# danieleschmidt/spin-torque-rl-gym

Hardware: AMD Instinct MI355X
Metric: env_steps_per_sec (higher is better)
Workload: dtype f64

## Files before the change

### spin-torque-rl-gym_amd/csrc/stg_kernels.hpp

```cpp
#pragma once
#include "../../include/spintorque_hip.h"
#include "stg_launch_plan.hpp"
#include "stg_physics.hpp"

#include <hip/hip_runtime.h>

#include <type_traits>

using namespace stg;

struct alignas(16) EnvRec {
    double m[3];
    double tgt[3];
    double etot;
    uint32_t stepw;
    uint32_t rng;
};
static_assert(sizeof(EnvRec) == 64, "state record size");
constexpr uint32_t STG_DONE_BIT = 0x80000000u;

struct StateView {
    EnvRec* rec;
};

// ... 557 lines not shown
            if (more && takers != 0ull) {
                const int n_take = (int)__builtin_popcountll(takers), first = (int)__builtin_ctzll(takers);
                const int rank = (int)__builtin_popcountll(takers & ((1ull << lane) - 1ull));
                const int64_t avail = loc_end - loc_q;
                const int need_new = n_take > avail ? (int)(n_take - avail) : 0;
                int64_t new_q = 0;
                const int new_stripe = stripe;
                if (need_new > 0 && queue_open) {
                    const int reserve = (takers == ~0ull && full_streak >= 1) ? 4 * 64 : need_new;
                    unsigned long long base = 0;
                    if (lane == first) base = atomicAdd(a.refill_cursor + stripe * REFILL_CURSOR_STRIDE, (unsigned long long)reserve);
                    base = (unsigned long long)__shfl((long long)base, first);
                    new_q = (int64_t)base;
                    const int64_t stripe_end = ((n_rest - stripe + REFILL_STRIPES - 1) / REFILL_STRIPES) * 64;
                    int64_t new_end = new_q + reserve;
                    if (new_end >= stripe_end) {
                        new_end = stripe_end;
                        const int64_t end_l = ((n_rest - lane + REFILL_STRIPES - 1) / REFILL_STRIPES) * 64;
                        const unsigned long long cur_l = __hip_atomic_load(a.refill_cursor + lane * REFILL_CURSOR_STRIDE, __ATOMIC_RELAXED, __HIP_MEMORY_SCOPE_AGENT);
                        unsigned long long open_s = __ballot((int64_t)cur_l < end_l);
                        open_s &= ~(1ull << stripe);
                        if (open_s == 0ull) queue_open = false;
                        else {
                            const unsigned long long after = stripe == 63 ? 0ull : (open_s >> (stripe + 1)) << (stripe + 1);
                            stripe = (int)__builtin_ctzll(after != 0ull ? after : open_s);
                        }
                    }
                    const bool from_old = rank < avail;
                    const int64_t q = from_old ? loc_q + rank : new_q + (rank - avail);
                    const int st = from_old ? loc_stripe : new_stripe;
                    const int64_t r = (q >> 6) * REFILL_STRIPES + st;
                    take((nw + r) * 64 + (q & 63), !has_env && r < n_rest && (from_old || q < new_end));
                    loc_q = new_q + need_new < new_end ? new_q + need_new : new_end;
                    loc_end = new_end;
                    loc_stripe = new_stripe;
                } else {
                    const int64_t q = loc_q + rank;
                    const int64_t r = (q >> 6) * REFILL_STRIPES + loc_stripe;
                    take((nw + r) * 64 + (q & 63), !has_env && q < loc_end && r < n_rest);
                    loc_q = loc_q + n_take < loc_end ? loc_q + n_take : loc_end;
                }
                more = queue_open || loc_q < loc_end;
                full_streak = takers == ~0ull ? full_streak + 1 : 0;
            }
        }
        if (__ballot(has_env) == 0ull && !more) break;
    }
}

template <int SOLVER, bool THERMAL, int MULTI, bool AXIS_Z, bool DEVPHYS, typename AT, bool PC, int WGW, bool IDS>
#ifndef STG_STEP_ATTR
#define STG_STEP_ATTR
#endif
__global__ void __launch_bounds__(PC ? 2 * WGW * 64 : WGW * 64, (SOLVER != STG_SOLVER_RK45 && !THERMAL && !DEVPHYS && AXIS_Z && MULTI != 2 && !(MULTI && WGW == 1)) ? 4 : 1) STG_STEP_ATTR
stg_step_kernel(const StepArgs a) {
#pragma clang fp contract(off)
    static_assert(!PC || THERMAL, "wave specialisation only exists for the thermal kernels");
    extern __shared__ double s_tab[];
    constexpr bool FIELD = SOLVER == STG_SOLVER_RK45;
    using NT = typename std::conditional<FIELD, double, float>::type;
    constexpr bool BARRIER = SOLVER != STG_SOLVER_RK4;
    constexpr int DEPTH = BARRIER ? 2 : 4;
    constexpr int RING = DEPTH * (FIELD ? SHARED_CHUNK_RK45 : SHARED_CHUNK_FIXED) * 64;
    static_assert(!PC || WGW == 1, "the wave-specialised form is one integrating + one producing wavefront");
    __shared__ NT s_norm[PC ? RING : 1];
    __shared__ int s_hs[2], s_go[2 * WGW];
    __shared__ unsigned long long s_cnt[(PC ? 2 : 1) * WGW * 3];
    __shared__ uint32_t s_rng[PC ? WGW * 64 : 1];
    const int lane = (int)(threadIdx.x & 63u);
    const int wave = __builtin_amdgcn_readfirstlane((int)(threadIdx.x >> 6));
    bool paired = PC;
    int64_t hyb_slot = 0;
    if (PC && a.hybrid) hyb_slot = stg_hybrid_block(blockIdx.x, wave, (uint32_t)(a.hybrid - 1), (a.N + TILE_ENVS - 1) / TILE_ENVS, paired);
    const bool producer = PC && paired && wave >= WGW;
    const int cw = producer ? (2 * WGW - 1 - wave) : (wave < WGW ? wave : wave - WGW);
    record_placement(a.placement, wave, lane, producer);
    const int64_t lane_slot = ((PC && a.hybrid) ? hyb_slot
                                                : stg_slot_block<WGW>(blockIdx.x, (uint32_t)((a.N + WGW * 64 - 1) / (WGW * 64)), a.perm != nullptr, cw, PC,
                                                                      (uint32_t)a.snake_rounds) * 64) + lane;
    const bool in_list = lane_slot < a.N;
    const int64_t o = in_list ? (a.perm ? (int64_t)a.perm[lane_slot] : lane_slot) : 0;
    const uint32_t id = (IDS && in_list) ? a.ids[o] : 0u;
    const bool bad = IDS && in_list && (int64_t)id >= a.n_state;
    if (bad && !producer) write_bad_id(a, o);
    const bool live = in_list && !bad;
    const int64_t i = IDS ? (live ? (int64_t)id : 0) : o;
    constexpr int ENV_LAYOUT = SOLVER == STG_SOLVER_RK45 ? ENV_LAYOUT_LLGS : (DEVPHYS ? ENV_LAYOUT_DEV : ENV_LAYOUT_CORE);
    double own_row[MULTI == 2 ? C_COUNT : 1];
    const double* row;
    if constexpr (MULTI == 2) {
        stg_device_params p;
        load_env_params<ENV_LAYOUT>(a.ep, i, p);
        derive_row(p, a.ep.gamma, a.ep.temperature, own_row);
        row = own_row;
    } else {
        row = class_row<MULTI != 0>(a.ctab, a.cls, a.ncls, i, live, s_tab, a.ep, ENV_LAYOUT);
    }
    if (!PC && !live) return;
    if (PC && !paired && !live) return;
    const int64_t N = a.N;
    const uint64_t env_id = (uint64_t)(a.env_id0 + i);

    if (producer) {
        constexpr int n_first = SOLVER == STG_SOLVER_RK45 ? SHARED_FIRST_RK45 : SHARED_CHUNK_FIXED;
        static_assert(3 * SHARED_SUBS3 == SHARED_CHUNK_FIXED, "chunk size of the 3-normal sub-steps");
        constexpr int n_chunk = SOLVER == STG_SOLVER_RK45 ? SHARED_CHUNK_RK45 : n_first;
        const double ghs = FIELD ? load_llgs(row).ghs : 0.0;
        for (int k = 0; k < a.K; ++k) {
            __syncthreads();
            const int p = (k & 1) * WGW;
            if (!any_flag<WGW>(lds_flag(s_go + p))) continue;
            const RngKey rk{a.c.seed, env_id, s_rng[cw * 64 + lane]};
            produce_normals<NT, FIELD, DEPTH, BARRIER>(s_norm, s_hs, lane, rk, n_first, n_chunk, ghs);
        }
        record_retired(a.placement, wave, lane, 0ull);
        return;
    }

    V3 m, tgt;
    double etot;
    int32_t step;
    uint32_t rng;
    bool done;
    load_state(a.s, i, m, tgt, etot, step, rng, done);
    const AT* act = (const AT*)a.actions;
    const Recorder norec{};
    unsigned long long c_steps = 0, c_sub = 0, c_noop = 0;

    for (int k = 0; k < a.K; ++k) {
        double J, T;
        if (k == 0 && a.perm) {
            typedef typename std::conditional<std::is_same<AT, double>::value, double2, float2>::type AT2;
            const AT2 aa = ((const AT2*)a.act_sorted)[live ? lane_slot : 0];
            parse_action<AT>(aa.x, aa.y, a.c.max_current, a.c.max_duration, J, T);
        } else {
            parse_action<AT>(act[((int64_t)k * 2 + 0) * N + o], act[((int64_t)k * 2 + 1) * N + o], a.c.max_current,
                             a.c.max_duration, J, T);
        }
        const bool last = (k == a.K - 1);
        const int64_t ko = a.out_every ? k : 0;
        const bool wr = (a.out_every || last) && live;
        const bool lane_solves = live && !(a.c.skip_done && done);
        const RngKey rk{a.c.seed, env_id, rng};
        SolveOut so{m, 0, 0, 0, false};
        if (PC && paired) {
            SharedNormalsT<NT, FIELD, DEPTH, BARRIER> shared{s_norm, s_hs, lane, 0, 0, 1};
            const int p = (k & 1) * WGW;
            s_rng[cw * 64 + lane] = rng;
            const bool mine = __ballot(lane_solves) != 0ull;
            s_go[p + cw] = mine ? 1 : 0;
            __syncthreads();
            if ((WGW == 1) ? mine : any_flag<WGW>(lds_flag(s_go + p))) {
                if (!BARRIER) s_hs[1] = 0;
                __syncthreads();
                so = run_solver<SOLVER, THERMAL, false, AXIS_Z, DEVPHYS>(m, J, T, row, a.c, rk, norec, shared, lane_solves);
            }
        }
        if (!(PC && paired) && lane_solves) {
            InlineNormals inl;
            so = run_solver<SOLVER, THERMAL, false, AXIS_Z, DEVPHYS>(m, J, T, row, a.c, rk, norec, inl, true);
        }
        env_step_tail(a, o, ko, wr, live, lane_solves, row, env_id, m, tgt, etot, step, rng, done, J, T, so, c_steps, c_sub, c_noop);
    }
    if (live) store_state(a.s, i, m, tgt, etot, step, rng, done);
    record_retired(a.placement, wave, lane, c_sub);
    const int ci = PC ? wave : cw;
    wave_add3(a.counters + (size_t)((blockIdx.x * (PC ? 2 : 1) * WGW + ci) % COUNTER_STRIPES) * COUNTER_STRIDE, s_cnt + ci * 3, c_steps, c_sub, c_noop);
}

template <bool THERMAL, bool MULTI, bool AXIS_Z, typename AT, int WGW, bool IDS>
__global__ void __launch_bounds__(WGW * 64) stg_step_refill_kernel(const StepArgs a) {
    extern __shared__ double s_tab[];
    __shared__ unsigned long long s_cnt[WGW * 3];
    const int lane = (int)(threadIdx.x & 63u);
    const int wave = __builtin_amdgcn_readfirstlane((int)(threadIdx.x >> 6));
    if (MULTI) {
        for (int j = threadIdx.x; j < a.ncls * C_COUNT; j += blockDim.x) s_tab[j] = a.ctab[j];
        __syncthreads();
    }
    const int64_t tiles = (a.N + TILE_ENVS - 1) / TILE_ENVS, nblk = tiles * TILE_WAVES, nw = a.refill_nw;
    const int64_t w = (int64_t)blockIdx.x * WGW + wave;
    record_placement(a.placement, wave, lane, false);
    if (w >= nw) return;
    unsigned long long c_steps = 0, c_sub = 0, c_noop = 0;
    refill_wave<THERMAL, MULTI, AXIS_Z, AT, IDS>(a, w, nw, 0, nblk, lane, s_tab, c_steps, c_sub, c_noop);
    refill_retire(a, w, nw, lane);
    record_retired(a.placement, wave, lane, c_sub);
    wave_add3(a.counters + (size_t)((blockIdx.x * WGW + wave) % COUNTER_STRIPES) * COUNTER_STRIDE, s_cnt + wave * 3, c_steps, c_sub, c_noop);
}

constexpr int64_t STG_WG4_MIN_ENVS = 65536;

template <class F>
static inline void with_flag(bool v, F&& f) {
    if (v) f(std::true_type{}); else f(std::false_type{});
}
template <class F>
static inline void with_multi(int multi, F&& f) {
    if (multi == 2) f(std::integral_constant<int, 2>{});
    else if (multi) f(std::integral_constant<int, 1>{});
    else f(std::integral_constant<int, 0>{});
}

template <int MULTI>
static size_t step_dyn_lds(const StepArgs& a) {
    return MULTI == 1 ? (size_t)a.ncls * C_COUNT * sizeof(double) : 0;
}

static inline unsigned step_grid(const StepArgs& a, int wgw) {
    const unsigned nwg = (unsigned)((a.N + wgw * 64 - 1) / (wgw * 64));
    if (!a.perm) return nwg;
    const unsigned tile_wgs = (unsigned)(TILE_WAVES / wgw);
    return ((nwg + tile_wgs - 1) / tile_wgs) * tile_wgs;
}

static int resident_workgroups_per_cu(const void* kernel, int block, size_t lds) {
    struct Key { const void* f; size_t lds; int v; };
    static thread_local Key cache[8] = {};
    static thread_local int used = 0;
    for (int j = 0; j < used; ++j) if (cache[j].f == kernel && cache[j].lds == lds) return cache[j].v;
    int nb = 0;
    if (hipOccupancyMaxActiveBlocksPerMultiprocessor(&nb, kernel, block, lds) != hipSuccess || nb < 1) nb = 2;
    if (used < 8) cache[used++] = Key{kernel, lds, nb};
    return nb;
}

static int32_t snake_rounds_of(const StepArgs& a, const void* kernel, int wgw, size_t lds) {
    if (!a.perm) return 0;
    const unsigned n_q = step_grid(a, wgw) / 8u;
    const int nb = resident_workgroups_per_cu(kernel, wgw * 64, lds);
    return (n_q > 32u && nb >= 2 && n_q <= 32u * (unsigned)nb + 16u) ? nb : 0;
}

template <int SOLVER, bool THERMAL, int MULTI, bool AXIS_Z, bool DEVPHYS, typename AT, bool PC, int WGW, bool IDS>
static void launch_step(const StepArgs& a, hipStream_t st) {
    if constexpr ((PC && (!THERMAL || DEVPHYS || WGW != 1)) || (DEVPHYS && SOLVER == STG_SOLVER_RK45)) return;
    else {
        const size_t lds = step_dyn_lds<MULTI>(a);
        StepArgs b = a;
        dim3 grid(step_grid(a, WGW));
        if constexpr (PC) {
            if (a.hybrid) grid = dim3(1024u);
            b.snake_rounds = (a.perm && step_grid(a, 1) / 8u <= 64u) ? 2 : 0;
        } else {
            b.snake_rounds = snake_rounds_of(a, (const void*)&stg_step_kernel<SOLVER, THERMAL, MULTI, AXIS_Z, DEVPHYS, AT, PC, WGW, IDS>, WGW, lds);
        }
        hipLaunchKernelGGL((stg_step_kernel<SOLVER, THERMAL, MULTI, AXIS_Z, DEVPHYS, AT, PC, WGW, IDS>), grid, dim3((PC ? 2 : 1) * WGW * 64), lds, st, b);
    }
}

template <int SOLVER, bool IDS>
static void dispatch_step(const StepArgs& a, bool thermal, int multi, bool axis_z, bool devphys, int act_f64, bool pc, hipStream_t st) {
    devphys = devphys && SOLVER != STG_SOLVER_RK45;
    pc = pc && thermal && !devphys;
    const bool wg4 = !pc && a.N >= STG_WG4_MIN_ENVS;
    with_flag(thermal, [&](auto THERMAL) { with_multi(multi, [&](auto MULTI) { with_flag(axis_z, [&](auto AXIS_Z) {
    with_flag(devphys, [&](auto DEVPHYS) { with_flag(act_f64 != 0, [&](auto F64) { with_flag(pc, [&](auto PC) { with_flag(wg4, [&](auto WG4) {
        using AT = std::conditional_t<F64.value, double, float>;
        launch_step<SOLVER, THERMAL.value, MULTI.value, AXIS_Z.value, DEVPHYS.value, AT, PC.value, WG4.value ? 4 : 1, IDS>(a, st);
    }); }); }); }); }); }); });
}

template <bool IDS>
static void dispatch_refill(const StepArgs& a, bool thermal, bool multi, bool axis_z, int act_f64, hipStream_t st) {
    constexpr int WGW = 4;
    const dim3 grid((unsigned)(((int64_t)a.refill_nw + WGW - 1) / WGW));
    with_flag(thermal, [&](auto THERMAL) { with_flag(multi, [&](auto MULTI) { with_flag(axis_z, [&](auto AXIS_Z) { with_flag(act_f64 != 0, [&](auto F64) {
        using AT = std::conditional_t<F64.value, double, float>;
        hipLaunchKernelGGL((stg_step_refill_kernel<THERMAL.value, MULTI.value, AXIS_Z.value, AT, WGW, IDS>), grid, dim3(WGW * 64),
                           step_dyn_lds<MULTI.value ? 1 : 0>(a), st, a);
    }); }); }); });
}

void stg_dispatch_step_rk4(const StepArgs& a, bool thermal, int multi, bool axis_z, bool devphys, int act_f64, bool pc, hipStream_t st);
void stg_dispatch_step_euler(const StepArgs& a, bool thermal, int multi, bool axis_z, bool devphys, int act_f64, bool pc, hipStream_t st);
void stg_dispatch_step_rk45(const StepArgs& a, bool thermal, int multi, bool axis_z, int act_f64, bool pc, hipStream_t st);
void stg_dispatch_step_rk45_refill(const StepArgs& a, bool thermal, bool multi, bool axis_z, int act_f64, hipStream_t st);
```

### spin-torque-rl-gym_amd/csrc/stg_physics.hpp

```cpp
#pragma once

#include <hip/hip_runtime.h>
#include <stdint.h>
#include <type_traits>

#include "stg_minstep.hpp"

namespace stg {

enum ClassConst : int {
    C_EX = 0, C_EY, C_EZ,
    C_HK,
    C_MS,
    C_ALPHA,
    C_GEFF,
    C_POL,
    C_MSV,
    C_HS_SIMPLE,
    C_RX, C_RY, C_RZ,
    C_DX, C_DY, C_DZ,
    C_HEX,
    C_BETA, C_BETAP,
    C_GAMMA,
    C_HS_LLGS,
// ... 71 lines not shown
#pragma clang fp contract(off)
    const double r = a - b;
    return r;
}

__device__ __forceinline__ double rsqrt_fast(double s) {
    const double y = __builtin_amdgcn_rsq(s);
    const double e = __builtin_fma(-(s * y), y, 1.0);
    return __builtin_fma(y * e, __builtin_fma(0.375, e, 0.5), y);
}

__device__ __forceinline__ void batch_ready(double at, double a0, double a1, double a2, double b0, double b1, double b2) {
    asm volatile("" : : "v"(at), "v"(a0), "v"(a1), "v"(a2), "v"(b0), "v"(b1), "v"(b2));
}

__device__ __forceinline__ double vgpr_const(double c) {
    asm volatile("" : "+v"(c));
    return c;
}

__device__ __forceinline__ double fmax_abs(double a, double b) {
    double r;
    asm("v_max_f64 %0, |%1|, |%2|" : "=v"(r) : "v"(a), "v"(b));
    return r;
}

__device__ __forceinline__ void commit_step(unsigned long long mask, double& d0, double s0, double& d1, double s1, double& d2, double s2,
                                            double& d3, double s3, double& d4, double s4, double& d5, double s5, double& d6, double s6) {
    unsigned long long saved;
    asm("s_and_saveexec_b64 %[sv], %[m]\n\t"
        "v_mov_b64 %[d0], %[s0]\n\t"
        "v_mov_b64 %[d1], %[s1]\n\t"
        "v_mov_b64 %[d2], %[s2]\n\t"
        "v_mov_b64 %[d3], %[s3]\n\t"
        "v_mov_b64 %[d4], %[s4]\n\t"
        "v_mov_b64 %[d5], %[s5]\n\t"
        "v_mov_b64 %[d6], %[s6]\n\t"
        "s_mov_b64 exec, %[sv]"
        : [d0] "+v"(d0), [d1] "+v"(d1), [d2] "+v"(d2), [d3] "+v"(d3), [d4] "+v"(d4), [d5] "+v"(d5), [d6] "+v"(d6), [sv] "=&s"(saved)
        : [s0] "v"(s0), [s1] "v"(s1), [s2] "v"(s2), [s3] "v"(s3), [s4] "v"(s4), [s5] "v"(s5), [s6] "v"(s6), [m] "s"(mask)
        : "scc");
}

__device__ __forceinline__ double rcp_fast(double x) {
    const double y = __builtin_amdgcn_rcp(x);
    return __builtin_fma(y, __builtin_fma(-x, y, 1.0), y);
}

__device__ __forceinline__ double inv_tenth_root(double e2, double tenth = 0.1) {
    const double y = (double)__builtin_amdgcn_exp2f(-0.1f * __builtin_amdgcn_logf((float)e2));
    const double y2 = y * y, y4 = y2 * y2, y8 = y4 * y4;
    const double e = __builtin_fma(-e2, y8 * y2, 1.0);
    return __builtin_fma(y * e, __builtin_fma(0.055, e, tenth), y);
}

__device__ __forceinline__ double fifth_root(double x) {
    int e;
    const double mant = frexp(x, &e);
    const double t = -0.2 * ((double)e + (double)__builtin_amdgcn_logf((float)mant));
    const double ti = rint(t);
    double r = ldexp((double)__builtin_amdgcn_exp2f((float)(t - ti)), (int)ti);
    const double r2 = r * r, r4 = r2 * r2;
    const double err = __builtin_fma(-x, r4 * r, 1.0);
    r = __builtin_fma(r * err, __builtin_fma(0.12, err, 0.2), r);
    const double q2 = r * r;
    return x * (q2 * q2);
}

__device__ __forceinline__ V3 cross(const V3& a, const V3& b) {
#pragma clang fp contract(off)
    return V3{__builtin_fma(a.y, b.z, -(a.z * b.y)), __builtin_fma(a.z, b.x, -(a.x * b.z)), __builtin_fma(a.x, b.y, -(a.y * b.x))};
}
__device__ __forceinline__ double dot(const V3& a, const V3& b) {
#pragma clang fp contract(off)
    return __builtin_fma(a.z, b.z, __builtin_fma(a.y, b.y, a.x * b.x));
}
__device__ __forceinline__ V3 scale3(double c, const V3& z) {
#pragma clang fp contract(off)
    return V3{c * z.x, c * z.y, c * z.z};
}
__device__ __forceinline__ bool finite3(const V3& a) { return isfinite(a.x) && isfinite(a.y) && isfinite(a.z); }

__device__ __forceinline__ void philox4x32_10(uint32_t c0, uint32_t c1, uint32_t c2, uint32_t c3, uint32_t k0,
                                              uint32_t k1, uint32_t (&out)[4]) {
#pragma unroll
    for (int r = 0; r < 10; ++r) {
        const uint32_t hi0 = __umulhi(0xD2511F53u, c0), lo0 = 0xD2511F53u * c0;
        const uint32_t hi1 = __umulhi(0xCD9E8D57u, c2), lo1 = 0xCD9E8D57u * c2;
        const uint32_t n0 = hi1 ^ c1 ^ k0, n2 = hi0 ^ c3 ^ k1;
        c0 = n0; c1 = lo1; c2 = n2; c3 = lo0;
        k0 += 0x9E3779B9u; k1 += 0xBB67AE85u;
    }
    out[0] = c0; out[1] = c1; out[2] = c2; out[3] = c3;
}

struct NormalStream {
    uint32_t s0, s1, s2, s3;
    float carry;
    __device__ __forceinline__ void init(uint64_t seed, uint64_t env_id, uint32_t env_step, uint32_t tag) {
        uint32_t r[4];
        philox4x32_10((uint32_t)env_id, (uint32_t)(env_id >> 32), env_step, tag, (uint32_t)seed, (uint32_t)(seed >> 32), r);
        s0 = r[0]; s1 = r[1]; s2 = r[2]; s3 = r[3] | 1u;
        carry = 0.0f;
    }
    __device__ __forceinline__ uint32_t next() {
        const uint32_t result = s0 + s3;
        const uint32_t t = s1 << 9;
        s2 ^= s0; s3 ^= s1; s1 ^= s2; s0 ^= s3; s2 ^= t;
        s3 = (s3 << 11) | (s3 >> 21);
        return result;
    }
    __device__ __forceinline__ float uniform() {
        return __uint_as_float(__builtin_amdgcn_alignbit(0x7fu, next(), 9u)) - 0.99999994f;
    }
    typedef float f32x2 __attribute__((ext_vector_type(2)));
    __device__ __forceinline__ void pair(float& a, float& b) {
        float t, c, s_;
        pair_head(t, c, s_);
        finish_pair(t, c, s_, a, b);
    }
    __device__ __forceinline__ void pair_head(float& t, float& c, float& s_) {
        f32x2 u{__uint_as_float(__builtin_amdgcn_alignbit(0x7fu, next(), 9u)), __uint_as_float(__builtin_amdgcn_alignbit(0x7fu, next(), 9u))};
        u = u - f32x2{0.99999994f, 0.99999994f};
        t = -1.3862943611198906f * __builtin_amdgcn_logf(u.x);
        c = __builtin_amdgcn_cosf(u.y);
        s_ = __builtin_amdgcn_sinf(u.y);
    }
    static __device__ __forceinline__ void finish_pair(float t, float c, float s_, float& a, float& b) {
        const float r = __builtin_amdgcn_sqrtf(t);
        const f32x2 cs = f32x2{c, s_} * f32x2{r, r};
        a = cs.x;
        b = cs.y;
    }
    __device__ __forceinline__ V3 draw3_even() {
        float a, b, c, d;
        pair(a, b);
        pair(c, d);
        carry = d;
        return V3{(double)a, (double)b, (double)c};
    }
    __device__ __forceinline__ V3 draw3_odd() {
        float a, b;
        pair(a, b);
        return V3{(double)carry, (double)a, (double)b};
    }
};

struct RngKey {
    uint64_t seed, env_id;
    uint32_t env_step;
};

struct InlineNormals {
    static constexpr bool kShared = false, kScaled = false;
    NormalStream ns;
    __device__ __forceinline__ void begin(const RngKey& rk) { ns.init(rk.seed, rk.env_id, rk.env_step, 0u); }
    __device__ __forceinline__ V3 draw(bool even) { return even ? ns.draw3_even() : ns.draw3_odd(); }
    static constexpr bool broken = false;
    __device__ __forceinline__ void peek() {}
    __device__ __forceinline__ bool chunk_end(bool lane_continues) { return lane_continues; }
    __device__ __forceinline__ bool chunk_end_wave(bool mine) { return mine; }
    __device__ __forceinline__ int32_t chunk_end_go(int32_t go) { return go; }
};

constexpr int SHARED_SUBS_RK4 = 2;
constexpr int SHARED_SUBS3 = 4 * SHARED_SUBS_RK4;
constexpr int SHARED_CHUNK_FIXED = 12 * SHARED_SUBS_RK4;
constexpr int SHARED_CHUNK_RK45 = 18;
constexpr int SHARED_TAIL_RK45 = 6;
constexpr int SHARED_FIRST_RK45 = 6 + SHARED_TAIL_RK45;
constexpr int PC_STOP = 1 << 30;
constexpr int PC_SPIN_CAP = 1 << 22;

typedef __attribute__((address_space(3))) int lds_int;
__device__ __forceinline__ volatile lds_int* lds_flag(const int* p) { return (volatile lds_int*)p; }

template <int WGW>
__device__ __forceinline__ bool any_flag(volatile lds_int* f) {
    int v = f[0];
#pragma unroll
    for (int j = 1; j < WGW; ++j) v |= f[j];
    return v != 0;
}
__device__ __forceinline__ int pc_load(const int* p) {
    return __builtin_amdgcn_readfirstlane(__hip_atomic_load(p, __ATOMIC_ACQUIRE, __HIP_MEMORY_SCOPE_WORKGROUP));
}
__device__ __forceinline__ void pc_store(int* p, int v) {
    __hip_atomic_store(p, v, __ATOMIC_RELEASE, __HIP_MEMORY_SCOPE_WORKGROUP);
}

template <typename T, bool SCALED, int DEPTH, bool BARRIER>
struct SharedNormalsT {
    static constexpr int CHUNK = SCALED ? SHARED_CHUNK_RK45 : SHARED_CHUNK_FIXED;
    static_assert(!BARRIER || DEPTH == 2, "the barrier form runs the producer exactly one chunk ahead");
    static constexpr bool kShared = true, kScaled = SCALED;
    const T* buf;
    int* hs;
    int lane, it, idx, seen;
    bool broken;
    static constexpr bool kToggle = BARRIER && SCALED;
    int slot_b, flag_b;
    __device__ __forceinline__ void begin(const RngKey&) {
        it = 0; idx = 0; seen = 1; broken = false;
        if (kToggle) {
            static_assert(((CHUNK * 64) & 63) == 0, "the slot bit and the lane bits are disjoint");
            slot_b = lane * (int)sizeof(T); flag_b = 0;
            asm volatile("" : "+v"(slot_b), "+v"(flag_b));
        }
    }
    __device__ __forceinline__ V3 draw(bool) {
        const T* b = kToggle ? (const T*)((const char*)buf + slot_b) + idx * 64 : buf + ((it & (DEPTH - 1)) * CHUNK + idx) * 64 + lane;
        idx += 3;
        return V3{(double)b[0], (double)b[64], (double)b[128]};
    }
    __device__ __forceinline__ void chunk_meet() {
        __syncthreads();
        slot_b ^= CHUNK * 64 * (int)sizeof(T);
        idx = 0;
    }
    __device__ __forceinline__ void seek_tail() { idx = CHUNK - SHARED_TAIL_RK45; }
    __device__ __forceinline__ void peek() {
        if (!BARRIER) seen = __hip_atomic_load(hs, __ATOMIC_RELAXED, __HIP_MEMORY_SCOPE_WORKGROUP);
    }
    __device__ __forceinline__ bool chunk_end(bool lane_continues) { return chunk_end_wave(__ballot(lane_continues) != 0ull); }
    __device__ __forceinline__ bool chunk_end_wave(bool mine) { return chunk_end_go(mine ? 1 : 0) != 0; }
    __device__ __forceinline__ int32_t chunk_end_go(int32_t go) {
        const bool mine = go != 0;
        if (kToggle) {
            *(volatile lds_int*)((volatile __attribute__((address_space(3))) char*)lds_flag(hs) + flag_b) = go;
            flag_b ^= (int)sizeof(int);
            if (!mine) __syncthreads();
            return go;
        }
        if (BARRIER) {
            lds_flag(hs)[it & 1] = go;
            __syncthreads();
            ++it;
            idx = 0;
            return go;
        }
        ++it;
        idx = 0;
        pc_store(hs + 1, it | (mine ? 0 : PC_STOP));
        int have = __builtin_amdgcn_readfirstlane(seen);
        if (__builtin_expect(mine && have <= it, 0)) {
            int spins = 0;
#pragma unroll 1
            do {
                if (spins) __builtin_amdgcn_s_sleep(1);
                have = pc_load(hs);
            } while (have <= it && ++spins <= PC_SPIN_CAP);
            broken = broken || have <= it;
        }
        seen = have;
        __builtin_amdgcn_fence(__ATOMIC_ACQUIRE, "workgroup");
        return (mine && !broken) ? 1 : 0;
    }
};

template <typename T, bool SCALED, int DEPTH, bool BARRIER>
__device__ __forceinline__ void produce_normals(T* buf, int* hs, int lane, const RngKey& rk, int n_first, int n_chunk, double c) {
    NormalStream ns;
    ns.init(rk.seed, rk.env_id, rk.env_step, 0u);
    bool even = true;
    auto fill = [&](int slot, int count) {
        T* b = buf + (slot * (SCALED ? SHARED_CHUNK_RK45 : SHARED_CHUNK_FIXED)) * 64 + lane;
        for (int j = 0; j < count; j += 3) {
            V3 z = even ? ns.draw3_even() : ns.draw3_odd();
            if (SCALED) z = scale3(c, z);
            even = !even;
            b[(j + 0) * 64] = (T)z.x; b[(j + 1) * 64] = (T)z.y; b[(j + 2) * 64] = (T)z.z;
        }
    };
    if constexpr (BARRIER && SCALED) {
        fill(0, n_first - SHARED_TAIL_RK45);
        T* ring = buf;
        buf += (SHARED_CHUNK_RK45 - SHARED_TAIL_RK45) * 64;
        fill(0, SHARED_TAIL_RK45);
        buf = ring;
    } else {
        fill(0, n_first);
    }
    if (!BARRIER) pc_store(hs, 1);
    __syncthreads();
    if (BARRIER) {
        for (int k = 1;; ++k) {
            fill(k & 1, n_chunk);
            __syncthreads();
            if (lds_flag(hs)[(k - 1) & 1] == 0) return;
        }
    }
    for (int k = 1;; ++k) {
        int v = pc_load(hs + 1);
#pragma unroll 1
        for (int spins = 0; (v & (PC_STOP - 1)) < k - DEPTH + 1 && !(v & PC_STOP); ++spins) {
            if (spins > PC_SPIN_CAP) return;
            __builtin_amdgcn_s_sleep(1);
            v = pc_load(hs + 1);
        }
        if (v & PC_STOP) return;
        fill(k & (DEPTH - 1), n_chunk);
        pc_store(hs, k + 1);
    }
}

struct SimpleK {
    V3 e;
    double ghk;
    double gdm;
    double alpha;
    double ghs;
};
__device__ __forceinline__ SimpleK make_simple(const V3& e, double hk, double ms, double alpha, double geff, double hs) {
#pragma clang fp contract(off)
    return SimpleK{e, -geff * hk, geff * ms, alpha, -geff * hs};
}
struct LlgsK {
    V3 r;
    V3 gd;
    double ghk, ghex;
    double alpha;
    double ghs;
    double gz;
    double agz;
};
__device__ __forceinline__ LlgsK make_llgs(const V3& r, const V3& d, double hk, double hex, double alpha, double gamma, double hs) {
#pragma clang fp contract(off)
    const double ng = -gamma;
    const double gz = ng * ((hk * r.z) * r.z + d.z);
    return LlgsK{r, V3{ng * d.x, ng * d.y, ng * d.z}, ng * hk, ng * hex, alpha, ng * hs, gz, alpha * gz};
}


template <bool THERMAL, bool AXIS_Z>
__device__ __forceinline__ V3 simple_rhs(const V3& m, const SimpleK& k, double ghk, double aJ, const V3& z) {
#pragma clang fp contract(off)
    if (AXIS_Z) {
        const double gz = (ghk + k.gdm) * m.z;
        V3 p;
        if (THERMAL) {
            const V3 g{k.ghs * z.x, k.ghs * z.y, __builtin_fma(k.ghs, z.z, gz)};
            p = cross(m, g);
        } else {
            p = V3{m.y * gz, -(m.x * gz), 0.0};
        }
        const double wx = __builtin_fma(k.alpha, p.x, aJ * m.y), wy = __builtin_fma(k.alpha, p.y, -(aJ * m.x));
        if (THERMAL) {
            const double wz = k.alpha * p.z;
            return V3{__builtin_fma(m.y, wz, __builtin_fma(-m.z, wy, p.x)), __builtin_fma(m.z, wx, __builtin_fma(-m.x, wz, p.y)),
                      __builtin_fma(m.x, wy, __builtin_fma(-m.y, wx, p.z))};
        }
        return V3{__builtin_fma(-m.z, wy, p.x), __builtin_fma(m.z, wx, p.y), __builtin_fma(m.x, wy, -(m.y * wx))};
    }
    const V3 t = cross(m, k.e);
    const double c = ghk * dot(m, k.e);
    const double d = k.gdm * m.z;
    V3 p;
    if (THERMAL) {
        const V3 g{__builtin_fma(k.ghs, z.x, c * k.e.x), __builtin_fma(k.ghs, z.y, c * k.e.y),
                   __builtin_fma(k.ghs, z.z, __builtin_fma(c, k.e.z, d))};
        p = cross(m, g);
    } else {
        p = V3{__builtin_fma(c, t.x, d * m.y), __builtin_fma(c, t.y, -(d * m.x)), c * t.z};
    }
    const V3 w{__builtin_fma(k.alpha, p.x, aJ * t.x), __builtin_fma(k.alpha, p.y, aJ * t.y),
               __builtin_fma(k.alpha, p.z, aJ * t.z)};
    return V3{__builtin_fma(m.y, w.z, __builtin_fma(-m.z, w.y, p.x)), __builtin_fma(m.z, w.x, __builtin_fma(-m.x, w.z, p.y)),
              __builtin_fma(m.x, w.y, __builtin_fma(-m.y, w.x, p.z))};
}

struct DevTorque {
    double sdl, sfl;
    V3 sigma;
    double ghk_pulse;
    bool any_sot;
};

__device__ __forceinline__ double vcma_keff(double volt, double ku, double xi, double td2, double vbd) {
    const double v = volt < -vbd ? -vbd : (volt > vbd ? vbd : volt);
    const double keff = ku + (-xi * fabs(v) / td2);
    return fmax(keff, -0.5 * ku);
}

template <bool THERMAL, bool AXIS_Z, bool DEVPHYS>
__device__ __forceinline__ V3 simple_stage(const V3& m, const SimpleK& k, double aJ, const V3& z, const DevTorque& dv,
                                           bool on) {
// ... 198 lines not shown
                  __builtin_fma(m.z, s, __builtin_fma(m.x, ht.y, __builtin_fma(-m.y, ht.x, -W.z)))};
    }
    const double c = k.ghk * dot(m, k.r);
    V3 g{(c * k.r.x + k.gd.x * m.x) + k.ghex * m.x, (c * k.r.y + k.gd.y * m.y) + k.ghex * m.y,
         (c * k.r.z + k.gd.z * m.z) + k.ghex * m.z};
    if (THERMAL) g = V3{g.x + ht.x, g.y + ht.y, g.z + ht.z};
    const V3 U{g.x, g.y, g.z + bpJ};
    const V3 W{k.alpha * g.x, k.alpha * g.y, __builtin_fma(k.alpha, g.z, bJ)};
    const double s = dot(m, W);
    return V3{__builtin_fma(m.x, s, __builtin_fma(m.y, U.z, __builtin_fma(-m.z, U.y, -W.x))),
              __builtin_fma(m.y, s, __builtin_fma(m.z, U.x, __builtin_fma(-m.x, U.z, -W.y))),
              __builtin_fma(m.z, s, __builtin_fma(m.x, U.y, __builtin_fma(-m.y, U.x, -W.z)))};
}

struct LlgsEnergyK {
    double kuv, edemag;
    V3 r, nfac;
};
__device__ __forceinline__ double llgs_energy(const V3& m, const LlgsEnergyK& k) {
    const double ct = dot(m, k.r);
    return -k.kuv * (ct * ct) + k.edemag * (k.nfac.x * (m.x * m.x) + k.nfac.y * (m.y * m.y) + k.nfac.z * (m.z * m.z));
}

__device__ __forceinline__ double llgs_torque_norms(const V3& m, double bJ, double bpJ) {
#pragma clang fp contract(off)
    const V3 mxp{m.y, -m.x, 0.0};
    const V3 mm = cross(m, mxp);
    const V3 a{bJ * mm.x, bJ * mm.y, bJ * mm.z}, b{bpJ * mxp.x, bpJ * mxp.y, bpJ * mxp.z};
    return sqrt((a.x * a.x + a.y * a.y) + a.z * a.z) + sqrt((b.x * b.x + b.y * b.y) + b.z * b.z);
}

__device__ __forceinline__ double rms3(const V3& a) { return sqrt(dot(a, a)) / 1.7320508075688772; }

struct Dp5Tab {
    double A51, A52, A53, A54, A61, A62, A63, A64, A65, E1, E3, E4, E5, E6, E7;
    double B4, third, c09, tenth;
};
__device__ __forceinline__ Dp5Tab make_dp5_tab() {
    Dp5Tab t;
    t.A51 = vgpr_const(19372.0 / 6561); t.A52 = vgpr_const(-25360.0 / 2187); t.A53 = vgpr_const(64448.0 / 6561); t.A54 = vgpr_const(-212.0 / 729);
    t.A61 = vgpr_const(9017.0 / 3168); t.A62 = vgpr_const(-355.0 / 33); t.A63 = vgpr_const(46732.0 / 5247); t.A64 = vgpr_const(49.0 / 176);
    t.A65 = vgpr_const(-5103.0 / 18656);
    t.E1 = vgpr_const(-71.0 / 57600); t.E3 = vgpr_const(71.0 / 16695); t.E4 = vgpr_const(-71.0 / 1920); t.E5 = vgpr_const(17253.0 / 339200);
    t.E6 = vgpr_const(-22.0 / 525); t.E7 = vgpr_const(1.0 / 40);
    t.B4 = vgpr_const(125.0 / 192); t.third = vgpr_const(1.0 / 3.0); t.c09 = vgpr_const(0.9); t.tenth = vgpr_const(0.1);
    return t;
}

struct LlgsLane {
    V3 y, f;
    V3 m0;
    double t, T, h_abs;
    double h_floor;
    double bJ, bpJ;
    int32_t attempts;
    int32_t npts;
    bool idle;
    bool rejected, active;
};

typedef unsigned long long lanemask;
struct LlgsMasks {
    lanemask active, pacc, low;
};
__device__ __forceinline__ bool lane_in(lanemask m) { return __builtin_amdgcn_inverse_ballot_w64(m); }
__device__ __forceinline__ LlgsMasks llgs_masks_open(const LlgsLane& L) {
    return LlgsMasks{__ballot(L.active), __ballot(!L.rejected), __ballot(L.h_abs < L.h_floor)};
}
__device__ __forceinline__ void llgs_masks_close(LlgsLane& L, const LlgsMasks& M) {
    L.active = lane_in(M.active);
    L.rejected = !lane_in(M.pacc);
}

template <bool RECORD>
__device__ __forceinline__ void llgs_lane_emit(LlgsLane& L, V3& out_m, const Recorder& rec, const LlgsEnergyK& ek) {
    const double inv = rsqrt_fast(dot(L.y, L.y));
    out_m = V3{L.y.x * inv, L.y.y * inv, L.y.z * inv};
    if (RECORD) rec.put(L.npts, L.t, out_m, rec.e ? llgs_energy(out_m, ek) : 0.0, rec.tq ? llgs_torque_norms(out_m, L.bJ, L.bpJ) : 0.0);
    ++L.npts;
}

template <bool THERMAL, bool AXIS_Z, bool CHECKED = true>
__device__ __forceinline__ V3 llgs_fun(const LlgsLane& L, const LlgsK& k, const V3& y, const V3& ht, bool on) {
    return llgs_rhs<THERMAL, AXIS_Z, CHECKED>(y, k, on ? L.bJ : 0.0, on ? L.bpJ : 0.0, ht);
}
template <bool THERMAL, class NSRC>
__device__ __forceinline__ V3 llgs_draw(NSRC& ns, const LlgsK& k, bool even) {
    if (!THERMAL) return V3{0.0, 0.0, 0.0};
    return NSRC::kScaled ? ns.draw(even) : scale3(k.ghs, ns.draw(even));
}

template <bool THERMAL, bool RECORD, bool AXIS_Z, class NSRC>
__device__ __forceinline__ void llgs_lane_begin(LlgsLane& L, V3& out_m, const V3& m0, double J, double T, const LlgsK& k, double beta,
                                                double betap, double rtol, double atol, double max_step, const RngKey& rk,
                                                const Recorder& rec, const LlgsEnergyK& ek, NSRC& ns, bool enabled) {
    const bool useJ = !(fabs(J) < 1e-12);
    L.bJ = useJ ? beta * J : 0.0;
    L.bpJ = useJ ? betap * J : 0.0;
    L.m0 = m0;
    L.T = T;
    if (THERMAL) ns.begin(rk);
    const double n0 = rsqrt_fast(dot(m0, m0));
    L.y = V3{m0.x * n0, m0.y * n0, m0.z * n0};
    L.t = 0.0;
    L.npts = 0;
    if (RECORD) llgs_lane_emit<RECORD>(L, out_m, rec, ek); else ++L.npts;
    L.f = llgs_fun<THERMAL, AXIS_Z>(L, k, L.y, llgs_draw<THERMAL>(ns, k, true), true);
    double h_abs;
    {
        const V3& y = L.y;
        const V3& f = L.f;
        const V3 sc{atol + fabs(y.x) * rtol, atol + fabs(y.y) * rtol, atol + fabs(y.z) * rtol};
        const V3 isc{rcp_fast(sc.x), rcp_fast(sc.y), rcp_fast(sc.z)};
        const double d0 = rms3(V3{y.x * isc.x, y.y * isc.y, y.z * isc.z});
        const double d1 = rms3(V3{f.x * isc.x, f.y * isc.y, f.z * isc.z});
        double h0 = (d0 < 1e-5 || d1 < 1e-5) ? 1e-6 : (0.01 * d0) * rcp_fast(d1);
        h0 = fmin(h0, T);
        const V3 y1{y.x + h0 * f.x, y.y + h0 * f.y, y.z + h0 * f.z};
        const V3 f1 = llgs_fun<THERMAL, AXIS_Z>(L, k, y1, llgs_draw<THERMAL>(ns, k, false), true);
        const double d2 = rms3(V3{(f1.x - f.x) * isc.x, (f1.y - f.y) * isc.y, (f1.z - f.z) * isc.z}) * rcp_fast(h0);
        const double h1 = (d1 <= 1e-15 && d2 <= 1e-15) ? fmax(1e-6, h0 * 1e-3) : fifth_root(0.01 * rcp_fast(fmax(d1, d2)));
        h_abs = fmin(fmin(100.0 * h0, h1), fmin(T, max_step));
    }
    L.rejected = false;
    L.attempts = 0;
    const double min_step = min_step_at(L.t);
    L.h_abs = h_abs > max_step ? max_step : (h_abs < min_step ? min_step : h_abs);
    L.h_floor = isfinite(T) ? min_step_at(T) : __builtin_inf();
    L.active = enabled && (L.t != T);
    L.idle = !L.active;
}

template <bool UNIFORM_IT>
__device__ __forceinline__ void llgs_lane_gate(LlgsLane& L, LlgsMasks& M, int32_t max_attempts) {
    if (__builtin_expect((M.low & M.active) != 0ull, 0)) {
        const double min_step = min_step_at(L.t);
        if (lane_in(M.pacc)) L.h_abs = L.h_abs < min_step ? min_step : L.h_abs;
        M.active &= ~__ballot(L.h_abs < min_step);
    }
    if (!UNIFORM_IT) M.active &= ~__ballot(L.attempts >= max_attempts);
}

__device__ __forceinline__ int32_t attempt_loop_next(lanemask& active, lanemask not_arrived, int32_t& it, int32_t budget) {
    int32_t go;
    asm("s_add_i32 %[it], %[it], 1\n\t"
        "s_and_b64 %[act], %[act], %[na]\n\t"
        "s_cselect_b32 %[go], %[bud], 0\n\t"
        "s_cmp_lt_i32 %[it], %[go]\n\t"
        "s_cselect_b32 %[go], 1, 0"
        : [act] "+s"(active), [it] "+s"(it), [go] "=&s"(go)
        : [na] "s"(not_arrived), [bud] "s"(budget)
        : "scc");
    return go;
}

template <bool THERMAL, bool RECORD, bool AXIS_Z, bool UNIFORM_IT, class NSRC>
__device__ __forceinline__ void llgs_lane_attempt(LlgsLane& L, LlgsMasks& M, V3& out_m, const LlgsK& k, const Dp5Tab& tb, double rtol,
                                                  double atol, double max_step, const Recorder& rec, const LlgsEnergyK& ek, NSRC& ns, V3& z2, V3& z3) {
    constexpr double A21 = 1.0 / 5;
    constexpr double A31 = 3.0 / 40, A32 = 9.0 / 40;
    constexpr double A41 = 44.0 / 45, A42 = -56.0 / 15, A43 = 32.0 / 9;
    constexpr double B1 = 35.0 / 384, B3 = 500.0 / 1113, B5 = -2187.0 / 6784, B6 = 11.0 / 84;
    const double B4 = tb.B4;
    const double A51 = tb.A51, A52 = tb.A52, A53 = tb.A53, A54 = tb.A54, A61 = tb.A61, A62 = tb.A62, A63 = tb.A63, A64 = tb.A64, A65 = tb.A65;
    const double E1 = tb.E1, E3 = tb.E3, E4 = tb.E4, E5 = tb.E5, E6 = tb.E6, E7 = tb.E7;
    const double T = L.T;
    const bool active = lane_in(M.active);
    const V3 y = L.y;
    const double t = L.t;
    auto fun = [&](const V3& yy, const V3& ht, bool on) -> V3 { return llgs_fun<THERMAL, AXIS_Z, false>(L, k, yy, ht, on); };
    auto draw = [&](bool even) -> V3 { return llgs_draw<THERMAL>(ns, k, even); };
    L.attempts += active ? 1 : 0;
    const double t_new = fmin(add_x(t, L.h_abs), T);
    const double h = sub_x(t_new, t);
    const double h_try = fabs(h);
    const bool on_end = add_x(t, h) <= T;
    const V3 k1 = L.f;
    constexpr bool BATCH = THERMAL && NSRC::kShared;
    if (THERMAL && !NSRC::kShared) { z2 = draw(true); z3 = draw(false); }
    V3 y2{y.x + (k1.x * A21) * h, y.y + (k1.y * A21) * h, y.z + (k1.z * A21) * h};
    if (BATCH) batch_ready(y2.z, z2.x, z2.y, z2.z, z3.x, z3.y, z3.z);
    const V3 k2 = fun(y2, z2, true);
    if constexpr (BATCH) ns.chunk_meet();
    V3 z4 = draw(true), z5{0.0, 0.0, 0.0};
    if (BATCH) { z5 = draw(false); __builtin_amdgcn_sched_barrier(0); }
    const V3 k3 = fun(V3{y.x + (k1.x * A31 + k2.x * A32) * h, y.y + (k1.y * A31 + k2.y * A32) * h,
                         y.z + (k1.z * A31 + k2.z * A32) * h}, z3, true);
    if (!BATCH) z5 = draw(false);
    V3 y4{y.x + (k1.x * A41 + k2.x * A42 + k3.x * A43) * h, y.y + (k1.y * A41 + k2.y * A42 + k3.y * A43) * h,
          y.z + (k1.z * A41 + k2.z * A42 + k3.z * A43) * h};
    if (BATCH) batch_ready(y4.z, z4.x, z4.y, z4.z, z5.x, z5.y, z5.z);
    const V3 k4 = fun(y4, z4, true);
    V3 z6 = draw(true), z7{0.0, 0.0, 0.0};
    if (BATCH) { z7 = draw(false); __builtin_amdgcn_sched_barrier(0); }
    const V3 k5 = fun(V3{y.x + (k1.x * A51 + k2.x * A52 + k3.x * A53 + k4.x * A54) * h,
                         y.y + (k1.y * A51 + k2.y * A52 + k3.y * A53 + k4.y * A54) * h,
                         y.z + (k1.z * A51 + k2.z * A52 + k3.z * A53 + k4.z * A54) * h}, z5, true);
    if (THERMAL) ns.peek();
    if (!BATCH) z7 = draw(false);
    V3 y6{y.x + (k1.x * A61 + k2.x * A62 + k3.x * A63 + k4.x * A64 + k5.x * A65) * h,
          y.y + (k1.y * A61 + k2.y * A62 + k3.y * A63 + k4.y * A64 + k5.y * A65) * h,
          y.z + (k1.z * A61 + k2.z * A62 + k3.z * A63 + k4.z * A64 + k5.z * A65) * h};
    if (BATCH) batch_ready(y6.z, z6.x, z6.y, z6.z, z7.x, z7.y, z7.z);
    const V3 k6 = fun(y6, z6, on_end);
    const V3 y_new{y.x + h * (k1.x * B1 + k3.x * B3 + k4.x * B4 + k5.x * B5 + k6.x * B6),
                   y.y + h * (k1.y * B1 + k3.y * B3 + k4.y * B4 + k5.y * B5 + k6.y * B6),
                   y.z + h * (k1.z * B1 + k3.z * B3 + k4.z * B4 + k5.z * B5 + k6.z * B6)};
    const V3 f_new = fun(y_new, z7, on_end);
    V3 z2n{0.0, 0.0, 0.0}, z3n{0.0, 0.0, 0.0};
    if constexpr (BATCH) { z2n = draw(true); z3n = draw(false); __builtin_amdgcn_sched_barrier(0); }
    const V3 ev{(k1.x * E1 + k3.x * E3 + k4.x * E4 + k5.x * E5 + k6.x * E6 + f_new.x * E7) * h,
                (k1.y * E1 + k3.y * E3 + k4.y * E4 + k5.y * E5 + k6.y * E6 + f_new.y * E7) * h,
                (k1.z * E1 + k3.z * E3 + k4.z * E4 + k5.z * E5 + k6.z * E6 + f_new.z * E7) * h};
    const V3 sc{atol + fmax_abs(y.x, y_new.x) * rtol, atol + fmax_abs(y.y, y_new.y) * rtol, atol + fmax_abs(y.z, y_new.z) * rtol};
    const V3 q{ev.x * rcp_fast(sc.x), ev.y * rcp_fast(sc.y), ev.z * rcp_fast(sc.z)};
    const double err2 = dot(q, q) * tb.third;
    const double err = err2;
    const lanemask accm = M.active & __ballot(err < 1.0);
    const bool acc = lane_in(accm);
    const double r9 = tb.c09 * inv_tenth_root(err, tb.tenth);
    const double fa = fmin(lane_in(M.pacc) ? 10.0 : 1.0, r9);
    const double fr = fmax(0.2, r9);
    double h_next = fmin(h_try * (acc ? fa : fr), max_step);
    M.low = __ballot(h_next < L.h_floor);
    L.h_abs = h_next;
    commit_step(accm, L.t, t_new, L.y.x, y_new.x, L.y.y, y_new.y, L.y.z, y_new.z, L.f.x, f_new.x, L.f.y, f_new.y, L.f.z, f_new.z);
    if (RECORD) { if (acc) llgs_lane_emit<RECORD>(L, out_m, rec, ek); } else L.npts += acc ? 1 : 0;
    M.pacc = accm;
    if (!UNIFORM_IT) M.active &= __ballot(L.t != T);
    if constexpr (BATCH) { z2 = z2n; z3 = z3n; }
}

template <bool RECORD, class NSRC>
__device__ __forceinline__ SolveOut llgs_lane_finish(LlgsLane& L, V3& out_m, const Recorder& rec, const LlgsEnergyK& ek, const NSRC& ns) {
    SolveOut o{L.m0, 0, 0, 0, false};
    if (!RECORD) { llgs_lane_emit<RECORD>(L, out_m, rec, ek); --L.npts; }
    o.m = out_m;
    o.n = L.npts - 1;
    o.work = L.attempts;
    const bool ok = L.idle || L.t == L.T;
    o.ok = ok && !ns.broken;
    if (!ok) o.m = L.m0;
    return o;
}

template <bool THERMAL, bool RECORD, bool AXIS_Z, class NSRC>
__device__ __forceinline__ SolveOut llgs_solve(const V3& m0, double J, double T, const LlgsK& k, double beta,
                                               double betap, double rtol, double atol, double max_step,
                                               int64_t max_attempts, const RngKey& rk, const Recorder& rec,
                                               const LlgsEnergyK& ek, NSRC& ns, bool enabled) {
    const Dp5Tab tb = make_dp5_tab();
    const V3 zero{0.0, 0.0, 0.0};
    LlgsLane L;
    V3 out_m = m0;
    llgs_lane_begin<THERMAL, RECORD, AXIS_Z>(L, out_m, m0, J, T, k, beta, betap, rtol, atol, max_step, rk, rec, ek, ns, enabled);
    LlgsMasks M = llgs_masks_open(L);
    atol = vgpr_const(atol);
    int32_t budget = (int32_t)max_attempts;
    asm volatile("" : "+s"(budget));
    int32_t it = 0;
    bool wave_go = M.active != 0ull;
    if (NSRC::kShared) wave_go = ns.chunk_end_wave(wave_go);
    V3 z2 = zero, z3 = zero;
    if constexpr (THERMAL && NSRC::kShared) {
        if (wave_go) { ns.seek_tail(); z2 = llgs_draw<THERMAL>(ns, k, true); z3 = llgs_draw<THERMAL>(ns, k, false); }
    }
    if (wave_go)
    for (;;) {
      llgs_lane_gate<true>(L, M, budget);
      llgs_lane_attempt<THERMAL, RECORD, AXIS_Z, true>(L, M, out_m, k, tb, rtol, atol, max_step, rec, ek, ns, z2, z3);
      if (!ns.chunk_end_go(attempt_loop_next(M.active, __ballot(L.t != L.T), it, budget))) break;
    }
    llgs_masks_close(L, M);
    return llgs_lane_finish<RECORD>(L, out_m, rec, ek, ns);
}

__device__ __forceinline__ double resistance(const V3& m_in, int dev_type, double r_p, double r_ap, double tmr,
                                             const V3& ref, double r_series) {
#pragma clang fp contract(off)
    if (dev_type == 0) {
        const double inv = rsqrt_fast(dot(m_in, m_in));
        const V3 m{m_in.x * inv, m_in.y * inv, m_in.z * inv};
        const double r = r_p * (1.0 + tmr * (1.0 - dot(m, ref)) * 0.5);
        return fmax(r, r_p * 0.5);
    }
    double r = r_p + (r_ap - r_p) * (1.0 - dot(m_in, ref)) * 0.5;
    if (dev_type == 1) r = r + r_series;
    return fmax(r, 1.0);
}

template <typename AT>
__device__ __forceinline__ void parse_action(AT a0, AT a1, double max_current, double max_duration, double& J, double& T) {
    const AT cmax = (AT)1e8, dmin = (AT)1e-12, dmax = (AT)1e-6;
    if (!isnan(a0)) a0 = a0 < -cmax ? -cmax : (a0 > cmax ? cmax : a0);
    if (!isnan(a1)) a1 = a1 < dmin ? dmin : (a1 > dmax ? dmax : a1);
    if (isnan(a0) || isnan(a1) || isinf(a0) || isinf(a1)) { a0 = (AT)0; a1 = dmin; }
    const double j = (double)a0, t = (double)a1;
    J = j < -max_current ? -max_current : (j > max_current ? max_current : j);
    T = t < 1e-12 ? 1e-12 : (t > max_duration ? max_duration : t);
}

__device__ __forceinline__ float obs_cast(double v) {
    const float f = (float)v;
    return isnan(f) ? 0.0f : (isinf(f) ? (f > 0 ? 1e6f : -1e6f) : f);
}

}
```

Measured before the change: 44.88 million.

## Replace per-chunk go-flag handshake with open/close ring protocol in barrier toggle mode

In the barrier-toggle shared-normals path, the solver wave no longer writes a go flag into LDS every attempt and no longer takes the entry handshake. The flag is set once when the solve opens and cleared once at the end (close), followed by a barrier. A new attempt_loop_more helper computes the continue condition with scalar instructions. This is meant to cut per-attempt LDS stores and branching in the hot loop, but it changes the consumer/producer coordination protocol, which risks mismatched barriers.

```diff
diff --git a/spin-torque-rl-gym_amd/csrc/stg_kernels.hpp b/spin-torque-rl-gym_amd/csrc/stg_kernels.hpp
--- a/spin-torque-rl-gym_amd/csrc/stg_kernels.hpp
+++ b/spin-torque-rl-gym_amd/csrc/stg_kernels.hpp
@@ -733,6 +733,7 @@
             __syncthreads();
             if ((WGW == 1) ? mine : any_flag<WGW>(lds_flag(s_go + p))) {
                 if (!BARRIER) s_hs[1] = 0;
+                if constexpr (BARRIER && FIELD) SharedNormalsT<NT, FIELD, DEPTH, BARRIER>::open(s_hs, lane);
                 __syncthreads();
                 so = run_solver<SOLVER, THERMAL, false, AXIS_Z, DEVPHYS>(m, J, T, row, a.c, rk, norec, shared, lane_solves);
             }
diff --git a/spin-torque-rl-gym_amd/csrc/stg_physics.hpp b/spin-torque-rl-gym_amd/csrc/stg_physics.hpp
--- a/spin-torque-rl-gym_amd/csrc/stg_physics.hpp
+++ b/spin-torque-rl-gym_amd/csrc/stg_physics.hpp
@@ -247,7 +247,7 @@
 };
 
 struct InlineNormals {
-    static constexpr bool kShared = false, kScaled = false;
+    static constexpr bool kShared = false, kScaled = false, kToggle = false;
     NormalStream ns;
     __device__ __forceinline__ void begin(const RngKey& rk) { ns.init(rk.seed, rk.env_id, rk.env_step, 0u); }
     __device__ __forceinline__ V3 draw(bool even) { return even ? ns.draw3_even() : ns.draw3_odd(); }
@@ -294,13 +294,14 @@
     int lane, it, idx, seen;
     bool broken;
     static constexpr bool kToggle = BARRIER && SCALED;
-    int slot_b, flag_b;
+    int slot_b;
+    int spare;
     __device__ __forceinline__ void begin(const RngKey&) {
         it = 0; idx = 0; seen = 1; broken = false;
         if (kToggle) {
             static_assert(((CHUNK * 64) & 63) == 0, "the slot bit and the lane bits are disjoint");
-            slot_b = lane * (int)sizeof(T); flag_b = 0;
-            asm volatile("" : "+v"(slot_b), "+v"(flag_b));
+            slot_b = lane * (int)sizeof(T);
+            asm volatile("" : "+v"(slot_b));
         }
     }
     __device__ __forceinline__ V3 draw(bool) {
@@ -313,6 +314,11 @@
         slot_b ^= CHUNK * 64 * (int)sizeof(T);
         idx = 0;
     }
+    static __device__ __forceinline__ void open(int* hs, int lane) { lds_flag(hs)[lane & 1] = 1; }
+    __device__ __forceinline__ void close(int32_t n) {
+        lds_flag(hs)[n & 1] = 0;
+        __syncthreads();
+    }
     __device__ __forceinline__ void seek_tail() { idx = CHUNK - SHARED_TAIL_RK45; }
     __device__ __forceinline__ void peek() {
         if (!BARRIER) seen = __hip_atomic_load(hs, __ATOMIC_RELAXED, __HIP_MEMORY_SCOPE_WORKGROUP);
@@ -321,12 +327,6 @@
     __device__ __forceinline__ bool chunk_end_wave(bool mine) { return chunk_end_go(mine ? 1 : 0) != 0; }
     __device__ __forceinline__ int32_t chunk_end_go(int32_t go) {
         const bool mine = go != 0;
-        if (kToggle) {
-            *(volatile lds_int*)((volatile __attribute__((address_space(3))) char*)lds_flag(hs) + flag_b) = go;
-            flag_b ^= (int)sizeof(int);
-            if (!mine) __syncthreads();
-            return go;
-        }
         if (BARRIER) {
             lds_flag(hs)[it & 1] = go;
             __syncthreads();
@@ -831,6 +831,16 @@
         : [na] "s"(not_arrived), [bud] "s"(budget)
         : "scc");
     return go;
+}
+__device__ __forceinline__ bool attempt_loop_more(lanemask& active, lanemask not_arrived, int32_t& it, int32_t budget) {
+    int32_t bound;
+    asm("s_add_i32 %[it], %[it], 1\n\t"
+        "s_and_b64 %[act], %[act], %[na]\n\t"
+        "s_cselect_b32 %[bd], %[bud], 0"
+        : [act] "+s"(active), [it] "+s"(it), [bd] "=&s"(bound)
+        : [na] "s"(not_arrived), [bud] "s"(budget)
+        : "scc");
+    return it < bound;
 }
 
 template <bool THERMAL, bool RECORD, bool AXIS_Z, bool UNIFORM_IT, class NSRC>
@@ -939,7 +949,8 @@
     asm volatile("" : "+s"(budget));
     int32_t it = 0;
     bool wave_go = M.active != 0ull;
-    if (NSRC::kShared) wave_go = ns.chunk_end_wave(wave_go);
+    constexpr bool RING = NSRC::kShared && NSRC::kToggle;
+    if (NSRC::kShared && !RING) wave_go = ns.chunk_end_wave(wave_go);
     V3 z2 = zero, z3 = zero;
     if constexpr (THERMAL && NSRC::kShared) {
         if (wave_go) { ns.seek_tail(); z2 = llgs_draw<THERMAL>(ns, k, true); z3 = llgs_draw<THERMAL>(ns, k, false); }
@@ -948,8 +959,11 @@
     for (;;) {
       llgs_lane_gate<true>(L, M, budget);
       llgs_lane_attempt<THERMAL, RECORD, AXIS_Z, true>(L, M, out_m, k, tb, rtol, atol, max_step, rec, ek, ns, z2, z3);
-      if (!ns.chunk_end_go(attempt_loop_next(M.active, __ballot(L.t != L.T), it, budget))) break;
-    }
+      const bool more = attempt_loop_more(M.active, __ballot(L.t != L.T), it, budget);
+      if constexpr (RING || !NSRC::kShared) { if (!more) break; }
+      else { if (!ns.chunk_end_go(more ? 1 : 0)) break; }
+    }
+    if constexpr (RING) ns.close(it);
     llgs_masks_close(L, M);
     return llgs_lane_finish<RECORD>(L, out_m, rec, ek, ns);
 }
```

New measurement: 45.54 million (median of 6 runs). +1.5%, better.
